# erikszasz/GaussianSplattingRegistration

Measured on AMD Instinct MI355X. Metric: Gaussians/sec through HEM level + ICP iters/sec, 2x5M-splat pair, higher is better.
Workload: dtype f32 (HEM) / f64 (ICP)

## Files before the change

### gaussiansplattingregistration_amd/csrc/hem.hip

```cpp
#include "gsr_common.h"
#include "gsr_math.h"
#include "gsr_normals.h"
#include "gsr_test_hooks.h"
#include "hem_device.h"
#include "hem_select.h"

#include <float.h>
#include <math.h>
#include <stdarg.h>
#include <stdlib.h>
#include <string.h>

#include <chrono>
#include <vector>

#include <rocprim/rocprim.hpp>

namespace gsr {

std::string& last_error() {
    static thread_local std::string s;
    return s;
}
int32_t fail(int32_t code, const char* fmt, ...) {
// ... 183 lines not shown
        const unsigned long long tot = __shfl(incl, 63);
        const unsigned long long cut = tot / 1000ull;
        int cl = 0, ch = 0;
        {
            unsigned long long run = incl - mine;
            for (int b = 0; b < HIST_BINS / 64; ++b) { run += hv[b]; cl += run <= cut ? 1 : 0; }
            run = tot - incl;
            for (int b = HIST_BINS / 64 - 1; b >= 0; --b) { run += hv[b]; ch += run <= cut ? 1 : 0; }
        }
        for (int o = 32; o > 0; o >>= 1) { cl += __shfl_xor(cl, o); ch += __shfl_xor(ch, o); }
        int lo = cl < HIST_BINS - 1 ? cl : HIST_BINS - 1;
        int hi = HIST_BINS - 1 - ch;
        hi = hi > lo ? hi : lo;
        lo = lo > 0 ? lo - 1 : 0;
        hi = hi < HIST_BINS - 1 ? hi + 1 : HIST_BINS - 1;
        const float w = ext / (float)HIST_BINS;
        const float nmn = mn[k] + w * (float)lo, nmx = mn[k] + w * (float)(hi + 1);
        mn[k] = nmn; mx[k] = nmx < mx[k] ? nmx : mx[k];
        inside *= 0.998;
    }
    float ex = mx[0] - mn[0], ey = mx[1] - mn[1], ez = mx[2] - mn[2];
    float emax = fmaxf(ex, fmaxf(ey, ez));
    float eps = emax * 1e-6f + 1e-30f;
    double vol = (double)(ex + eps) * (double)(ey + eps) * (double)(ez + eps);
    double c = cbrt(vol * (double)target / (inside > 1.0 ? inside : 1.0));
    if (!(c > 0.0)) c = 1.0;
    int gx, gy, gz;
    for (;;) {
        double fx = floor(ex / c) + 1.0, fy = floor(ey / c) + 1.0, fz = floor(ez / c) + 1.0;
        if (fx * fy * fz <= (double)max_cells && fx < 2e6 && fy < 2e6 && fz < 2e6) { gx = (int)fx; gy = (int)fy; gz = (int)fz; break; }
        c *= 1.2599210498948732;
    }
    g.ox = mn[0]; g.oy = mn[1]; g.oz = mn[2];
    g.c = (float)c; g.inv_c = 1.0f / g.c;
    g.slack = 1e-5f * (emax + g.c);
    g.gx = gx; g.gy = gy; g.gz = gz; g.ncells = gx * gy * gz;
    if (lane == 0) *gp = g;
}

__global__ __launch_bounds__(256) void k_keys(int64_t n, const float* __restrict__ xyz,
                                              const GridParams* __restrict__ gpp,
                                              unsigned* __restrict__ keys, unsigned* __restrict__ idx) {
    const GridParams g = *gpp;
    for (int64_t i = (int64_t)blockIdx.x * blockDim.x + threadIdx.x; i < n; i += (int64_t)gridDim.x * blockDim.x) {
        int cx = cell_of(xyz[3 * i], g.ox, g.inv_c, g.gx);
        int cy = cell_of(xyz[3 * i + 1], g.oy, g.inv_c, g.gy);
        int cz = cell_of(xyz[3 * i + 2], g.oz, g.inv_c, g.gz);
        keys[i] = (unsigned)((cz * g.gy + cy) * g.gx + cx);
        idx[i] = (unsigned)i;
    }
}

template <typename OffT>
__global__ __launch_bounds__(256) void k_run_starts(int64_t m, const unsigned* __restrict__ skeys, int64_t nkeys,
                                                    OffT* __restrict__ start) {
    for (int64_t j = (int64_t)blockIdx.x * blockDim.x + threadIdx.x; j < m; j += (int64_t)gridDim.x * blockDim.x) {
        unsigned k = skeys[j];
        int64_t prev = j == 0 ? -1 : (int64_t)skeys[j - 1];
        if ((int64_t)k != prev)
            for (int64_t c = prev + 1; c <= (int64_t)k; ++c) start[c] = (OffT)j;
        if (j == m - 1)
            for (int64_t c = (int64_t)k + 1; c <= nkeys; ++c) start[c] = (OffT)m;
    }
}
template <typename OffT>
__global__ void k_fill_const(int64_t n, OffT* p, OffT v) {
    for (int64_t j = (int64_t)blockIdx.x * blockDim.x + threadIdx.x; j < n; j += (int64_t)gridDim.x * blockDim.x) p[j] = v;
}

__global__ __launch_bounds__(256) void k_gather(int64_t n, const unsigned* __restrict__ order, const float4* __restrict__ rec, float delta,
                                                float4* __restrict__ A, float4* __restrict__ geo, float* __restrict__ Rs,
                                                int* __restrict__ pflag, int* __restrict__ iflag,
                                                const float* __restrict__ sh, int F, float* __restrict__ sh_tail ) {
    __shared__ float4 s_t[4][64 * 5];
    float4* st = s_t[threadIdx.x >> 6];
    const int lane = threadIdx.x & 63;
    if (blockIdx.x == 0 && threadIdx.x == 0) iflag[n] = 0;
    if (sh_tail && blockIdx.x == 0)
        for (int t = threadIdx.x; t < ((F + 3) & ~3) + 4; t += blockDim.x) sh_tail[t] = t < F ? sh[(n - 1) * F + t] : 0.0f;
    const int64_t base = (int64_t)blockIdx.x * blockDim.x + (threadIdx.x & ~63);
    if (base < n) {
        const int64_t j = base + lane;
        const unsigned oi = j < n ? order[j] : 0u;
        float4 v[4];
        unsigned iu[4];
#pragma unroll
        for (int u = 0; u < 4; ++u) {
            iu[u] = (unsigned)__shfl((int)oi, (lane >> 2) + 16 * u, 64);
            v[u] = rec[4 * (int64_t)iu[u] + (lane & 3)];
        }
        asm volatile("" : "+v"(v[0].x), "+v"(v[0].y), "+v"(v[0].z), "+v"(v[0].w), "+v"(v[1].x), "+v"(v[1].y), "+v"(v[1].z), "+v"(v[1].w),
                          "+v"(v[2].x), "+v"(v[2].y), "+v"(v[2].z), "+v"(v[2].w), "+v"(v[3].x), "+v"(v[3].y), "+v"(v[3].z), "+v"(v[3].w));
        if ((lane & 3) == 0) {
#pragma unroll
            for (int u = 0; u < 4; ++u) v[u].w = __uint_as_float((__float_as_uint(v[u].w) & 3u) | (iu[u] << 2));
        }
#pragma unroll
        for (int u = 0; u < 4; ++u) {
            const int r = (lane >> 2) + 16 * u;
            if (base + r < n) {
                geo[4 * (base + r) + (lane & 3)] = v[u];
                st[r * 5 + (lane & 3)] = v[u];
            }
        }
        __builtin_amdgcn_wave_barrier();
        if (j < n) {
            const float4 a = st[lane * 5], b = st[lane * 5 + 1], cc = st[lane * 5 + 2];
            const unsigned fl = __float_as_uint(a.w);
            A[j] = a;
            float R = 0.0f;
            if (fl & 1u) {
                const s6 cov = {b.x, b.y, b.z, b.w, cc.x, cc.y};
                R = delta * sqrtf(eig_max6(cov));
            }
            Rs[j] = R;
            pflag[j] = (int)(fl & 1u);
            iflag[j] = (fl & 2u) ? 0 : 1;
        }
        __builtin_amdgcn_wave_barrier();
    }
}
struct __attribute__((packed, aligned(4))) f4u { float x, y, z, w; };
__global__ __launch_bounds__(256) void k_gather_sh(int64_t n, int F, int RSH, const unsigned* __restrict__ order,
                                                   const float* __restrict__ sh, float* __restrict__ shs,
                                                   const int64_t* __restrict__ poff, const unsigned* __restrict__ pcnt, int P, int policy, float thr,
                                                   int* __restrict__ mode_out) {
    {
        int direct = policy == 1 ? 1 : 0;
        if (policy == 2) {
            const double pairs = P > 0 ? (double)poff[P - 1] + (double)pcnt[P - 1] : 0.0;
            direct = pairs < (double)thr * (double)n ? 1 : 0;
        }
        if (blockIdx.x == 0 && threadIdx.x == 0) *mode_out = direct;
        if (direct) return;
    }
    const int Q = RSH >> 2;
    const int64_t total = n * Q;
    const int64_t stride = (int64_t)gridDim.x * blockDim.x;
    auto row_piece = [&](int64_t t, int64_t& j, int& q) -> float4 {
        j = total < ((int64_t)1 << 31) ? (int64_t)((unsigned)t / (unsigned)Q) : t / Q;
        q = (int)(t - j * Q);
        const float* src = sh + (int64_t)order[j] * F + 4 * q;
        const int left = F - 4 * q;
        float4 v;
        if (left >= 4) {
            const f4u u = *reinterpret_cast<const f4u*>(src);
            v = make_float4(u.x, u.y, u.z, u.w);
        } else {
            v.x = left > 0 ? src[0] : 0.0f; v.y = left > 1 ? src[1] : 0.0f; v.z = left > 2 ? src[2] : 0.0f; v.w = 0.0f;
        }
        return v;
    };
    int64_t t = (int64_t)blockIdx.x * blockDim.x + threadIdx.x;
    for (; t + stride < total; t += 2 * stride) {
        int64_t j0, j1;
        int q0, q1;
        const float4 v0 = row_piece(t, j0, q0), v1 = row_piece(t + stride, j1, q1);
        reinterpret_cast<float4*>(shs + j0 * RSH)[q0] = v0;
        reinterpret_cast<float4*>(shs + j1 * RSH)[q1] = v1;
    }
    if (t < total) {
        int64_t j0;
        int q0;
        const float4 v0 = row_piece(t, j0, q0);
        reinterpret_cast<float4*>(shs + j0 * RSH)[q0] = v0;
    }
}
__global__ __launch_bounds__(256) void k_scatter_list(int64_t n, const int* __restrict__ flag, const int* __restrict__ pos,
                                                      unsigned* __restrict__ list) {
    for (int64_t j = (int64_t)blockIdx.x * blockDim.x + threadIdx.x; j < n; j += (int64_t)gridDim.x * blockDim.x)
        if (flag[j]) list[pos[j]] = (unsigned)j;
}

__global__ __launch_bounds__(256) void k_child_stream(int64_t n, int64_t cells, int P, const float4* __restrict__ A, const int* __restrict__ pflag,
                                                      const int* __restrict__ ppos, const int* __restrict__ cellStart,
                                                      float4* __restrict__ Ac, int* __restrict__ cellStartC, int pad,
                                                      const int* __restrict__ irank , int* __restrict__ cellStartI) {
    const int64_t stride = (int64_t)gridDim.x * blockDim.x, t0 = (int64_t)blockIdx.x * blockDim.x + threadIdx.x;
    for (int64_t t = t0; t < pad; t += stride) Ac[(n - P) + t] = make_float4(0.0f, 0.0f, 0.0f, 0.0f);
    for (int64_t j = t0; j < n; j += stride) {
        if (pflag[j]) continue;
        const float4 a = A[j];
        Ac[j - ppos[j]] = make_float4(a.x, a.y, a.z, __uint_as_float(((unsigned)j << 2) | (__float_as_uint(a.w) & 3u)));
    }
    for (int64_t cidx = t0; cidx <= cells; cidx += stride) {
        const int sidx = cellStart[cidx];
        cellStartC[cidx] = sidx - (sidx < n ? ppos[sidx] : P);
        if (irank) cellStartI[cidx] = irank[sidx];
    }
}

#ifndef ORDER_AXIS_BITS
#define ORDER_AXIS_BITS 6
#endif
#ifndef ORDER_FINE_FROM
#define ORDER_FINE_FROM 1000000
#endif
__host__ __device__ inline int order_axis_bits(int P) { return P >= ORDER_FINE_FROM ? ORDER_AXIS_BITS : 3; }
__host__ __device__ inline int order_drop_bits(int P) { return P >= ORDER_FINE_FROM ? 0 : 1; }
__host__ __device__ inline int order_key_bits(int P) { return 3 * order_axis_bits(P) - order_drop_bits(P); }
__global__ __launch_bounds__(1024) void k_heavy_items(int P, const unsigned* __restrict__ sorted_keys, int* __restrict__ nheavy_p,
                                                      const unsigned* __restrict__ porder,
                                                      const unsigned* __restrict__ pcap, const int64_t* __restrict__ coff, unsigned* __restrict__ part_out,
                                                      int own_lo, int own_hi, int first_pull, int max_items,
                                                      uint2* __restrict__ hitem, int* __restrict__ hfirst, unsigned* __restrict__ pcnt,
                                                      int* __restrict__ hq, int* __restrict__ error_flag) {
    __shared__ int s_wsum[16];
    __shared__ int s_base, s_nheavy;
    unsigned part = SEL_PART;
    {
        const unsigned long long cand = (unsigned long long)coff[P - 1] + pcap[P - 1];
        while (part > 2048u && (unsigned long long)part * 4ull * 7168ull > cand) part >>= 1;
    }
    if (threadIdx.x == 0) {
        *part_out = part;
        int lo = 0, hi = P;
        while (lo < hi) { const int mid = (lo + hi) >> 1; if (sorted_keys[mid] >= (3u << order_key_bits(P))) hi = mid; else lo = mid + 1; }
        s_nheavy = lo;
        *nheavy_p = lo;
        s_base = 0;
    }
    __syncthreads();
    const int nheavy = s_nheavy;
    const int lane = threadIdx.x & 63, wv = threadIdx.x >> 6;
    for (int h0 = 0; h0 < nheavy; h0 += 1024) {
        const int h = h0 + (int)threadIdx.x;
        int p = -1, np = 0;
        if (h < nheavy) {
            p = (int)porder[h];
            if (p >= own_lo && p < own_hi) { const unsigned c = pcap[p]; np = (int)(c / part + (c % part ? 1u : 0u)); np = np < 1 ? 1 : np; }
        }
        int incl = np;
        for (int o = 1; o < 64; o <<= 1) { const int v = __shfl_up(incl, o, 64); if (lane >= o) incl += v; }
        if (lane == 63) s_wsum[wv] = incl;
// ... 1457 lines not shown
        const int64_t row0 = t * a.tile;
        const int nrows = (int)(n_pre - row0 < a.tile ? n_pre - row0 : a.tile);
        const int k0 = holes_below(s_holes, d, row0), k1 = holes_below(s_holes, d, row0 + nrows);
        if (k1 == 0) continue;
        const int kn = row0 + nrows < n_pre ? k1 : 0;
        const int tail0 = nrows - kn;
        __syncthreads();
        if ((int)threadIdx.x < nrows) {
            const int64_t r = row0 + threadIdx.x;
            int k = 0; bool hole = false;
            for (int i = 0; i < d; ++i) { k += (int64_t)s_holes[i] < r ? 1 : 0; hole = hole || (int64_t)s_holes[i] == r; }
            s_k[threadIdx.x] = hole ? (short)-1 : (short)(k - k0);
        }
        __syncthreads();
        const int ndst = nrows - (k1 - k0);
        const float* hn = a.halo + (t + 1) * ERASE_MAX * a.W;
        int off = 0;
        for (int q = 0; q < 6; ++q) {
            const int w = a.w[q];
            if (w > 0) {
                float* arr = a.arr[q];
                for (unsigned e = threadIdx.x; e < (unsigned)(nrows * w); e += blockDim.x) {
                    const unsigned rl = e / (unsigned)w, cc = e - rl * (unsigned)w;
                    const int kk = s_k[rl];
                    if (kk < 0) continue;
                    const float v = (int)rl >= tail0 ? hn[off + ((int)rl - tail0) * w + cc] : arr[(row0 + rl) * w + cc];
                    s_stage[((int)rl - kk) * w + cc] = v;
                }
                __syncthreads();
                for (int e = threadIdx.x; e < ndst * w; e += blockDim.x) arr[(row0 - k0) * w + e] = s_stage[e];
                __syncthreads();
            }
            off += ERASE_MAX * w;
        }
        {
            uint8_t* sb = reinterpret_cast<uint8_t*>(s_stage);
            if ((int)threadIdx.x < nrows && s_k[threadIdx.x] >= 0) {
                const int rl = threadIdx.x;
                sb[rl - s_k[rl]] = rl >= tail0 ? halo_b[(t + 1) * ERASE_MAX + (rl - tail0)] : a.flags[row0 + rl];
            }
            __syncthreads();
            if ((int)threadIdx.x < ndst) a.flags[row0 - k0 + threadIdx.x] = sb[threadIdx.x];
            __syncthreads();
        }
    }
}

__global__ void k_level_tail(int64_t n, int P, const int* __restrict__ orank_in, const int* __restrict__ oflag_in, long long out_cap,
                             long long* __restrict__ lvl, int* __restrict__ abort_p) {
    long long n_orph = (long long)orank_in[n - 1] + oflag_in[n - 1];
    if ((long long)P + n_orph > out_cap) { *abort_p = 1; n_orph = out_cap > P ? out_cap - P : 0; }
    lvl[0] = (long long)P + n_orph;
    lvl[1] = n_orph;
}

struct LevelCollect {
    const int64_t* coff; const unsigned* pcap;
    const int64_t* poff; const unsigned* pcnt;
    int P;
    const int* cnt;
    const long long* lvl;
    const GridParams* gp; const unsigned* bbox;
};
enum { LC_CAND = 0, LC_PAIRS, LC_ORPHANS, LC_NPRE, LC_FLAGS, LC_HEAVY, LC_ITEMS, LC_MAXPAIRS, LC_DROPPED, LC_NEXT_P, LC_NEXT_IRR, LC_NEXT_GP, LC_WORDS = 16 };
__global__ void k_level_collect(LevelCollect q, unsigned long long* __restrict__ dst, unsigned long long seq) {
    const int t = threadIdx.x;
    unsigned long long v = 0ull;
    const bool sel = q.P > 0 && q.coff != nullptr;
    if (t == LC_CAND) v = sel ? (unsigned long long)q.coff[q.P - 1] + q.pcap[q.P - 1] : 0ull;
    else if (t == LC_PAIRS) v = sel ? (unsigned long long)q.poff[q.P - 1] + q.pcnt[q.P - 1] : 0ull;
    else if (t == LC_ORPHANS) v = q.lvl ? (unsigned long long)q.lvl[1] : 0ull;
    else if (t == LC_NPRE) v = q.lvl ? (unsigned long long)q.lvl[0] : 0ull;
    else if (t == LC_FLAGS) v = (q.cnt[2] ? 1ull : 0ull) | (q.cnt[12] ? 2ull : 0ull) | (q.cnt[13] ? 4ull : 0ull);
    else if (t == LC_HEAVY) v = (unsigned)q.cnt[8];
    else if (t == LC_ITEMS) v = (unsigned)q.cnt[10];
    else if (t == LC_MAXPAIRS) v = (unsigned)q.cnt[15];
    else if (t == LC_DROPPED) v = (unsigned)q.cnt[3];
    else if (t == LC_NEXT_P) v = q.bbox[6];
    else if (t == LC_NEXT_IRR) v = q.bbox[7];
    else if (t < LC_WORDS) v = reinterpret_cast<const unsigned long long*>(q.gp)[t - LC_NEXT_GP];
    if (t < LC_WORDS) __hip_atomic_store(dst + 16 + t, v, __ATOMIC_RELAXED, __HIP_MEMORY_SCOPE_SYSTEM);
    __threadfence_system();
    __syncthreads();
    if (t == 0) __hip_atomic_store(dst + 15, seq, __ATOMIC_RELEASE, __HIP_MEMORY_SCOPE_SYSTEM);
}
__global__ __launch_bounds__(256) void k_compact_rows(int64_t n, int width, const int* __restrict__ keep,
                                                      const int* __restrict__ pos, const float* __restrict__ src,
                                                      float* __restrict__ dst) {
    const int64_t total = n * width;
    for (int64_t t = (int64_t)blockIdx.x * blockDim.x + threadIdx.x; t < total; t += (int64_t)gridDim.x * blockDim.x) {
        const int64_t i = t / width;
        if (keep[i]) dst[(int64_t)pos[i] * width + (t - i * width)] = src[t];
    }
}
__global__ __launch_bounds__(256) void k_compact_rows4(int64_t n, int width, const int* __restrict__ keep,
                                                       const int* __restrict__ pos, const float* __restrict__ src,
                                                       float* __restrict__ dst) {
    const int Q = (width + 3) >> 2;
    const int64_t total = n * Q;
    for (int64_t t = (int64_t)blockIdx.x * blockDim.x + threadIdx.x; t < total; t += (int64_t)gridDim.x * blockDim.x) {
        const int64_t i = total < ((int64_t)1 << 31) ? (int64_t)((unsigned)t / (unsigned)Q) : t / Q;
        if (!keep[i]) continue;
        const int q = (int)(t - i * Q);
        const float* s4 = src + i * width + 4 * q;
        float* d4 = dst + (int64_t)pos[i] * width + 4 * q;
        const int left = width - 4 * q;
// ... 967 lines not shown
        long long dg = 0;
        GSR_HIP(hipMemcpyAsync(&dg, c->pcounts.p, 8, hipMemcpyDeviceToHost, st));
        GSR_HIP(hipStreamSynchronize(st));
        if (dg > 0) {
            const int64_t words = (n_pre_glob + 31) / 32 + 1;
            GSR_TRY(c->gbits.reserve((size_t)words * 4)); GSR_TRY(c->wcnt.reserve((size_t)words * 4)); GSR_TRY(c->wpre.reserve((size_t)words * 4));
            GSR_HIP(hipMemsetAsync(c->gbits.p, 0, (size_t)words * 4, st));
            if (n_pre > 0) {
                GSR_TRY(c->scratch.reserve((size_t)n_pre * 4));
                hipLaunchKernelGGL(k_not_flag, dim3(stride_grid(n_pre)), blk, 0, st, n_pre, c->keep.as<int>(), c->scratch.as<int>());
                hipLaunchKernelGGL(k_bits_set, dim3(stride_grid(n_pre)), blk, 0, st, n_pre, c->gid_next.as<unsigned>(), c->scratch.as<int>(), c->gbits.as<unsigned>());
            }
            GSR_TRY(gsr_comm_allreduce(c->comm, c->gbits.p, words, GSR_DT_U32, GSR_OP_SUM, (void*)st));
            hipLaunchKernelGGL(k_bits_popc, dim3(stride_grid(words)), blk, 0, st, words, c->gbits.as<unsigned>(), c->wcnt.as<int>());
            GSR_TRY(exclusive_scan<int>(c, c->wcnt.as<int>(), c->wpre.as<int>(), words));
            if (dropped > 0) {
                GSR_TRY(c->grank.reserve((size_t)n_pre * 4));
                hipLaunchKernelGGL(k_compact_u32, dim3(stride_grid(n_pre)), blk, 0, st, n_pre, c->keep.as<int>(), c->kpos.as<int>(), c->gid_next.as<unsigned>(), c->grank.as<unsigned>());
                c->gid_next.swap(c->grank);
            }
            if (O.n > 0) hipLaunchKernelGGL(k_gid_drop, dim3(stride_grid(O.n)), blk, 0, st, O.n, c->gbits.as<unsigned>(), c->wpre.as<int>(), c->gid_next.as<unsigned>());
            n_glob_next = n_pre_glob - dg;
        }
        c->part_stats[6] = dg;
        return GSR_OK;
    }
};

}

namespace {

constexpr int32_t GSR_RETRY_SYNC = -1000;

struct LevelRun {
    gsr_hem_ctx* c;
    hipStream_t st;
    Level& L;
    Level& O;
    const bool dbg_sync, part, sharded;
    bool spec = false;
    const int sh_policy;
    const int64_t n_own;
    int64_t n;
    const int F, RSH;
    PartLevel pl;
    const dim3 blk{256};
    dim3 grd;
    GridParams gp;
    int P_all = 0, P = 0, n_irr = 0;
    int* cnt = nullptr;
    long long* lvl = nullptr;
    const float4* rec_src = nullptr;
    bool ranks_forked = false, sh_pending = false, sh_launched = false, flags_forked = false;
    SelectArgs sa;
    size_t Pm = 1;
    int own_lo = 0, own_hi = 0;
    int64_t M = 0;
    unsigned long long cand = 0, cap_pairs = 0;
    const int64_t* seg = nullptr;
    const unsigned* pc = nullptr;
    const float* pw = nullptr;
    int bshift = 0, nbuckets = 0;
    int* overflow_flag = nullptr;
    bool fixed_tried = false;
    int64_t n_orph = 0, n_pre = 0, out_cap = 0;
    bool out_active = false;
    uint64_t rng_pos0 = 0;
    int64_t dropped = 0, P_glob = 0, O_glob = 0, n_pre_glob = 0, n_glob_next = 0;
    float pro_ms = 0.0f;

    LevelRun(gsr_hem_ctx* ctx, bool allow_async)
        : c(ctx), st(ctx->stream), L(ctx->cur), O(ctx->nxt), dbg_sync(getenv("GSR_HEM_DEBUG_SYNC") != nullptr), part(ctx->comm != nullptr),
          sharded(ctx->shard_world > 1 && ctx->shard_allreduce != nullptr), sh_policy(ctx->comm == nullptr ? ctx->sh_policy : 0), n_own(ctx->cur.n), n(ctx->cur.n), F(ctx->cur.F), RSH((ctx->cur.F + 3) & ~3) {
        spec = allow_async;
        pl.c = c; pl.st = st; pl.n_own = n_own;
        memset(&sa, 0, sizeof(sa));
    }
    ~LevelRun() {
        if (out_active) for (int i = 0; i < 5; ++i) { DevBuf* b = level_big(c->nxt, i); b->p = nullptr; b->cap = 0; b->swap(c->spare_out[i]); }
    }

    int32_t run(int64_t* n_out, int64_t* n_dropped);
    int32_t grid_phase();
    int32_t select_phase();
    int32_t sums_phase();
    int32_t sums_fixed();
    int32_t sums_exact();
    int32_t compact_pairs();
    int32_t output_ranks();
    int32_t open_output();
    int32_t mstep_phase();
    int32_t flags_and_validity();
    int32_t compact_erased(int64_t n_keep);
    int32_t erase_in_place(int64_t rows_bound, bool may_allocate, int64_t alloc_rows = 0);
    bool erase_on_device = false;
    int32_t launch_gather_sh(bool fork);
    int32_t widen_scan(const unsigned* cnt_in, int64_t* off, int64_t count);
    int32_t total_of(const int64_t* off, const unsigned* cnt_in, int64_t count, int64_t* out);
};

struct WidenU32 { __device__ __host__ int64_t operator()(unsigned v) const { return (int64_t)v; } };
int32_t LevelRun::widen_scan(const unsigned* cnt_in, int64_t* off, int64_t count) {
    auto in = rocprim::make_transform_iterator(cnt_in, WidenU32());
    size_t bytes = 0;
    if (count >= GSR_SCAN_BIG_N) {
        GSR_HIP(rocprim::exclusive_scan<scan_cfg64_big>(nullptr, bytes, in, off, (int64_t)0, (size_t)count, rocprim::plus<int64_t>(), st));
// ... 30 lines not shown
                           c->ghost_sh.as<float>(), c->shs.as<float>());
    else
        hipLaunchKernelGGL(k_gather_sh, dim3(shg), blk, 0, sst, n, F, RSH, c->order.as<unsigned>(), L.sh.as<float>(), c->shs.as<float>(),
                           P > 0 ? c->poff.as<int64_t>() : (const int64_t*)nullptr, c->pcnt.as<unsigned>(), P, sh_policy, c->sh_direct_pairs,
                           reinterpret_cast<int*>(lvl + 3));
    if (fork) { GSR_HIP(hipEventRecord(c->ev_sh_join, c->aux2)); sh_pending = true; }
    return GSR_OK;
}

int32_t LevelRun::grid_phase() {
    GSR_TRY(c->counters.reserve(128)); GSR_TRY(c->lvl.reserve(64));
    lvl = c->lvl.as<long long>();
    if (!part && !sharded) {
        if (!(c->pro.valid && c->pro.n == n)) GSR_TRY(prologue_now(c));
        if (!c->pro.valid) return fail(GSR_E_INVALID, "gsr_hem_run_level: no prologue for the level");
        gp = c->pro.gp; P_all = c->pro.P; n_irr = c->pro.n_irr; c->cblock = c->pro.cblock; pro_ms = c->pro.ms;
        c->pro.valid = false;
        cnt = c->counters.as<int>() + 16 * c->cblock;
    } else {
        c->pro.valid = false;
        c->cblock ^= 1;
        cnt = c->counters.as<int>() + 16 * c->cblock;
        GSR_TRY(c->rec.reserve(n * 64)); GSR_TRY(c->bbox.reserve(64));
        GSR_TRY(c->gparams.reserve(sizeof(GridParams)));
        GSR_TRY(c->bbox_part.reserve((size_t)grd.x * 8 * 4)); GSR_TRY(c->hist.reserve(3 * HIST_BINS * 4));
        hipLaunchKernelGGL(k_prep, grd, blk, 0, st, n, L.xyz.as<float>(), L.color.as<float>(), L.cov6.as<float>(), L.opacity.as<float>(),
                           L.weight.as<float>(), L.is_parent.as<uint8_t>(), c->rec.as<float4>(), c->bbox_part.as<unsigned>(), (const long long*)nullptr);
        hipLaunchKernelGGL(k_bbox_reduce, dim3(1), dim3(256), 0, st, (int)grd.x, c->bbox_part.as<unsigned>(), c->bbox.as<unsigned>(),
                           (unsigned*)cnt, 16, c->hist.as<unsigned>(), 3 * HIST_BINS, (unsigned*)nullptr, 0);
        if (part) {
            hipLaunchKernelGGL(k_flip3, dim3(1), dim3(64), 0, st, c->bbox.as<unsigned>());
            GSR_TRY(gsr_comm_allreduce(c->comm, c->bbox.p, 6, GSR_DT_U32, GSR_OP_MAX, (void*)st));
            hipLaunchKernelGGL(k_flip3, dim3(1), dim3(64), 0, st, c->bbox.as<unsigned>());
        }
        hipLaunchKernelGGL(k_hist, dim3(stride_grid(n) > 512 ? 512 : stride_grid(n)), blk, 0, st, n, L.xyz.as<float>(), c->bbox.as<unsigned>(), c->hist.as<unsigned>(),
                           (const long long*)nullptr);
        if (part) GSR_TRY(gsr_comm_allreduce(c->comm, c->hist.p, 3 * HIST_BINS, GSR_DT_U32, GSR_OP_SUM, (void*)st));
        hipLaunchKernelGGL(k_grid_params, dim3(1), dim3(64), 0, st, c->bbox.as<unsigned>(), c->hist.as<unsigned>(), part ? c->n_global : n, c->cell_target,
                           c->max_cells, c->gparams.as<GridParams>(), (const long long*)nullptr);
        static_assert(sizeof(GridParams) == 40, "GridParams is read back as five 8-byte words");
        Collect q;
        q.n = 7;
        for (int i = 0; i < 5; ++i) { q.src[i] = (const char*)c->gparams.p + 8 * i; q.bytes[i] = 8; }
        q.src[5] = c->bbox.as<unsigned>() + 6; q.src[6] = c->bbox.as<unsigned>() + 7;
        q.bytes[5] = q.bytes[6] = 4;
        unsigned long long w[8];
        GSR_TRY(read_back(c, q, w));
        memcpy(&gp, w, sizeof(gp));
        P_all = (int)(unsigned)w[5]; n_irr = (int)(unsigned)w[6];
    }
    overflow_flag = cnt + 12;
    c->stats[5] = gp.ncells;
    GSR_TRY(c->pflag_in.reserve(n * 4)); GSR_TRY(c->oflag_in.reserve(n * 4)); GSR_TRY(c->prank_in.reserve(n * 4)); GSR_TRY(c->orank_in.reserve(n * 4));
    if (!part && c->aux && c->ev_pre) {
        GSR_HIP(hipEventRecord(c->ev_fork, st)); GSR_HIP(hipStreamWaitEvent(c->aux, c->ev_fork, 0));
        hipLaunchKernelGGL(k_flags_in, grd, blk, 0, c->aux, n, n_own, L.is_parent.as<uint8_t>(), c->pflag_in.as<int>(), c->oflag_in.as<int>());
        GSR_TRY(exclusive_scan<int>(c, c->pflag_in.as<int>(), c->prank_in.as<int>(), n, true));
        GSR_HIP(hipEventRecord(c->ev_pre, c->aux));
        ranks_forked = true;
    }

    rec_src = c->rec.as<float4>();
    if (part) {
        GSR_TRY(pl.halo(gp, L, F, n));
        grd = dim3(stride_grid(n));
        rec_src = c->rec_loc.as<float4>();
    }
    GSR_TRY(c->keys.reserve(n * 4)); GSR_TRY(c->idx.reserve(n * 4)); GSR_TRY(c->skeys.reserve(n * 4)); GSR_TRY(c->order.reserve(n * 4));
    if (part) {
        GSR_TRY(c->perm.reserve(n * 4));
        hipLaunchKernelGGL(k_iota, grd, blk, 0, st, n, c->idx.as<unsigned>());
        GSR_TRY(sort_pairs<unsigned>(c, c->gid_loc.as<unsigned>(), c->skeys.as<unsigned>(), c->idx.as<unsigned>(), c->perm.as<unsigned>(), n, bits_for(c->n_global + 1)));
        hipLaunchKernelGGL(k_keys_rec, grd, blk, 0, st, n, rec_src, c->perm.as<unsigned>(), c->gparams.as<GridParams>(), c->keys.as<unsigned>(), c->idx.as<unsigned>());
    } else
        hipLaunchKernelGGL(k_keys, grd, blk, 0, st, n, L.xyz.as<float>(), c->gparams.as<GridParams>(), c->keys.as<unsigned>(), c->idx.as<unsigned>());
    GSR_TRY(sort_pairs<unsigned>(c, c->keys.as<unsigned>(), c->skeys.as<unsigned>(), c->idx.as<unsigned>(), c->order.as<unsigned>(), n,
                                 bits_for(gp.ncells)));
    GSR_TRY(c->cellStart.reserve(((size_t)gp.ncells + 1) * 4));
    hipLaunchKernelGGL(k_run_starts<int>, grd, blk, 0, st, n, c->skeys.as<unsigned>(), (int64_t)gp.ncells, c->cellStart.as<int>());

    GSR_TRY(c->A.reserve((n + SEL_PAD) * 16)); GSR_TRY(c->geo.reserve((size_t)n * 64));
    if (sh_policy != 1) GSR_TRY(c->shs.reserve((size_t)n * (RSH > 0 ? RSH : 1) * 4));
    GSR_TRY(c->Rs.reserve(n * 4)); GSR_TRY(c->pflag.reserve(n * 4));
    GSR_TRY(c->iflag.reserve((n + 1) * 4)); GSR_TRY(c->irank.reserve((n + 1) * 4)); GSR_TRY(c->ipos.reserve(n * 4)); GSR_TRY(c->ppos.reserve(n * 4)); GSR_TRY(c->plist.reserve(n * 4));
    const bool tail = !part && F > 0;
    if (tail) GSR_TRY(c->sh_tail.reserve((size_t)(RSH + 4) * 4));
    hipLaunchKernelGGL(k_gather, dim3((unsigned)((n + 255) / 256)), blk, 0, st, n, c->order.as<unsigned>(), rec_src, c->delta, c->A.as<float4>(), c->geo.as<float4>(),
                       c->Rs.as<float>(), c->pflag.as<int>(), c->iflag.as<int>(), L.sh.as<float>(), F, tail ? c->sh_tail.as<float>() : (float*)nullptr);
    if (part && F > 0) {
        hipLaunchKernelGGL(k_fill_const<int>, dim3(1), dim3(1), 0, st, (int64_t)1, reinterpret_cast<int*>(lvl + 3), 0);
        GSR_TRY(launch_gather_sh(true)); sh_launched = true;
    }
    GSR_TRY(exclusive_scan<int>(c, c->pflag.as<int>(), c->ppos.as<int>(), n));
    if (part) {
        GSR_TRY(c->pown.reserve(n * 4)); GSR_TRY(c->ppos_own.reserve(n * 4)); GSR_TRY(c->inv.reserve(n * 4));
        hipLaunchKernelGGL(k_own_flags, grd, blk, 0, st, n, n_own, c->order.as<unsigned>(), c->pflag.as<int>(), c->pown.as<int>(), c->inv.as<unsigned>());
        GSR_TRY(exclusive_scan<int>(c, c->pown.as<int>(), c->ppos_own.as<int>(), n));
        hipLaunchKernelGGL(k_scatter_list, grd, blk, 0, st, n, c->pown.as<int>(), c->ppos_own.as<int>(), c->plist.as<unsigned>());
    } else
        hipLaunchKernelGGL(k_scatter_list, grd, blk, 0, st, n, c->pflag.as<int>(), c->ppos.as<int>(), c->plist.as<unsigned>());
    if (part || n_irr > 0) {
        GSR_TRY(exclusive_scan<int>(c, c->iflag.as<int>(), c->irank.as<int>(), n + 1));
        hipLaunchKernelGGL(k_scatter_list, grd, blk, 0, st, n, c->iflag.as<int>(), c->irank.as<int>(), c->ipos.as<unsigned>());
    }
    P = P_all;
    if (part) {
        Collect q;
        q.n = 5;
        q.src[0] = c->irank.as<int>() + n; q.src[1] = c->ppos.as<int>() + (n - 1); q.src[2] = c->pflag.as<int>() + (n - 1);
        q.src[3] = c->ppos_own.as<int>() + (n - 1); q.src[4] = c->pown.as<int>() + (n - 1);
        for (int i = 0; i < 5; ++i) q.bytes[i] = 4;
        unsigned long long w[8];
        GSR_TRY(read_back(c, q, w));
        n_irr = (int)w[0];
        P_all = (int)w[1] + (int)w[2];
        P = (int)w[3] + (int)w[4];
    }
    c->stats[0] = P;
    c->stats_ex[0] = n_irr;
    GSR_TRY(c->Ac.reserve(((size_t)(n - P_all) + SEL_PAD) * 16)); GSR_TRY(c->cellStartC.reserve(((size_t)gp.ncells + 1) * 4));
    const bool have_irr = part || n_irr > 0;
    if (have_irr) GSR_TRY(c->cellStartI.reserve(((size_t)gp.ncells + 1) * 4));
    hipLaunchKernelGGL(k_child_stream, grd, blk, 0, st, n, (int64_t)gp.ncells, P_all, c->A.as<float4>(), c->pflag.as<int>(), c->ppos.as<int>(),
                       c->cellStart.as<int>(), c->Ac.as<float4>(), c->cellStartC.as<int>(), (int)SEL_PAD,
                       have_irr ? c->irank.as<int>() : (const int*)nullptr, c->cellStartI.as<int>());
    GSR_CHECKPOINT("grid + gather");
    GSR_TIME(c->ev[1], st);
    return GSR_OK;
}

int32_t LevelRun::select_phase() {
    Pm = (size_t)(P > 0 ? P : 1);
    GSR_TRY(c->pcnt.reserve(Pm * 4)); GSR_TRY(c->pcap.reserve(Pm * 4)); GSR_TRY(c->poff.reserve((Pm + 1) * 8));
    GSR_TRY(c->scratch.reserve((Pm * 2 + 128) * 8));
    sa.A = c->A.as<float4>(); sa.geo = c->geo.as<float4>();
    sa.Rs = c->Rs.as<float>(); sa.plist = c->plist.as<unsigned>(); sa.cellStart = c->cellStart.as<int>();
    sa.gp = c->gparams.as<GridParams>(); sa.P = P;
    sa.Ac = c->Ac.as<float4>(); sa.cellStartC = c->cellStartC.as<int>(); sa.cellStartI = c->cellStartI.as<int>();
    sa.irank = c->irank.as<int>(); sa.ipos = c->ipos.as<unsigned>(); sa.n_irr = n_irr; sa.ell = c->use_ell ? 1 : 0;
    own_lo = sharded ? (int)((int64_t)P * c->shard_rank / c->shard_world) : 0;
    own_hi = sharded ? (int)((int64_t)P * (c->shard_rank + 1) / c->shard_world) : P;
    sa.own_lo = own_lo; sa.own_hi = own_hi;
    {
        const float t = c->kappa * c->kappa * 0.5f;
        float x;
        if (t != t) x = t;
        else if (t < 0.0f) x = -1.0f;
        else if (t > FLT_MAX) x = t;
        else {
            x = t * t;
            if (x > FLT_MAX) x = FLT_MAX;
            while (x < FLT_MAX && sqrtf(nextafterf(x, INFINITY)) <= t) x = nextafterf(x, INFINITY);
            while (x > 0.0f && sqrtf(x) > t) x = nextafterf(x, -INFINITY);
        }
        sa.colorThr2 = x;
    }
    sa.kldThr = c->delta * c->delta * 0.5f;
    sa.tau2 = c->tau * c->tau;
    sa.pcnt = c->pcnt.as<unsigned>();
    sa.pcap = c->pcap.as<unsigned>();
    sa.part_p = reinterpret_cast<const unsigned*>(lvl + 2);
    sa.abort_p = cnt + 2;
    sa.np = c->select_np > 0 ? c->select_np : (P >= SEL_NP * 7168 ? SEL_NP : (P >= 2 * 7168 ? 2 : 1));
    M = 0;
    constexpr int WPB = SEL_WPB;
#define GSR_LAUNCH_SELECT(MODE) GSR_TRY(launch_select(MODE, sa, st, c->aux, c->ev_fork, c->ev_join))
    c->sparse_path = false;
    if (P > 0) {
        GSR_TRY(c->prec.reserve(Pm * sizeof(ParentRec)));
        launch_parent_prep(st, P, c->plist.as<unsigned>(), c->geo.as<float4>(), c->Rs.as<float>(), sa.kldThr, sa.ell, c->prec.as<ParentRec>());
        sa.prec = c->prec.as<ParentRec>();
        if (c->use_rowlist && Pm * 2 * SEL_ROWS * sizeof(int2) <= c->rowlist_max) {
            GSR_TRY(c->rowlist.reserve(Pm * 2 * SEL_ROWS * sizeof(int2)));
            sa.rowlist = c->rowlist.as<int2>();
        }
        launch_spans(st, sa);
        GSR_TRY(c->coff.reserve((Pm + 1) * 8));
        GSR_TRY(widen_scan(c->pcap.as<unsigned>(), c->coff.as<int64_t>(), P));
// ... 326 lines not shown
            hipLaunchKernelGGL(k_mstep_heavy_finish, dim3(256), dim3(64), 0, st, ma);                                    \
        }                                                                                                                \
    }
        GSR_TIME1(c->evm[0], st);
        if (nq == 0) { GSR_LAUNCH_MSTEP(0) }
        else if (nq <= 1 * MSTEP_NV) { GSR_LAUNCH_MSTEP(1) }
        else if (nq <= 2 * MSTEP_NV) { GSR_LAUNCH_MSTEP(2) }
        else if (nq <= 4 * MSTEP_NV) { GSR_LAUNCH_MSTEP(4) }
        else if (nq <= 8 * MSTEP_NV) { GSR_LAUNCH_MSTEP(8) }
        else if (nq <= 16 * MSTEP_NV) { GSR_LAUNCH_MSTEP(16) }
        else { GSR_LAUNCH_MSTEP(32) }
#undef GSR_LAUNCH_MSTEP
        if (msplit && hst != st) GSR_HIP(hipStreamWaitEvent(st, c->ev_mjoin, 0));
        GSR_TIME1(c->evm[1], st);
    }
    hipLaunchKernelGGL(k_orphan_rows, dim3(stride_grid(n_own)), blk, 0, st, n_own, P, c->oflag_in.as<int>(), c->orank_in.as<int>(), L.xyz.as<float>(), L.color.as<float>(),
                       L.cov6.as<float>(), L.opacity.as<float>(), L.weight.as<float>(), L.sh.as<float>(), F, O.xyz.as<float>(), O.color.as<float>(),
                       O.cov6.as<float>(), O.opacity.as<float>(), O.weight.as<float>(), O.sh.as<float>(), (int64_t)(spec ? out_cap : n_pre));
    if (sharded && P > 0) {
        const int W = c->shard_world, RW = 14 + F;
        const int chunk = (P + W - 1) / W + 1;
        const size_t chunk_bytes = (size_t)chunk * RW * 4;
        GSR_TRY(c->shard_send.reserve(chunk_bytes)); GSR_TRY(c->shard_recv.reserve(chunk_bytes * W));
        const int own_cnt = own_hi - own_lo;
        if (own_cnt > 0)
            hipLaunchKernelGGL((k_shard_rows<true>), dim3(stride_grid((int64_t)own_cnt * RW)), blk, 0, st, own_lo, own_cnt, F, c->plist.as<unsigned>(),
                               c->order.as<unsigned>(), c->prank_in.as<int>(), c->shard_send.as<float>(), O.xyz.as<float>(), O.color.as<float>(),
                               O.cov6.as<float>(), O.opacity.as<float>(), O.weight.as<float>(), O.sh.as<float>());
        GSR_HIP(hipStreamSynchronize(st));
        if (c->shard_allgather(c->shard_send.p, c->shard_recv.p, (int64_t)chunk_bytes, c->shard_user) != 0)
            return fail(GSR_E_INVALID, "gsr_hem_run_level: all-gather callback failed (merged components)");
        for (int r = 0; r < W; ++r) {
            if (r == c->shard_rank) continue;
            const int lo = (int)((int64_t)P * r / W), hi = (int)((int64_t)P * (r + 1) / W);
            if (hi > lo)
                hipLaunchKernelGGL((k_shard_rows<false>), dim3(stride_grid((int64_t)(hi - lo) * RW)), blk, 0, st, lo, hi - lo, F, c->plist.as<unsigned>(),
                                   c->order.as<unsigned>(), c->prank_in.as<int>(), c->shard_recv.as<float>() + (size_t)r * chunk * RW, O.xyz.as<float>(),
                                   O.color.as<float>(), O.cov6.as<float>(), O.opacity.as<float>(), O.weight.as<float>(), O.sh.as<float>());
        }
    }
    P_glob = P; O_glob = n_orph;
    if (part) GSR_TRY(pl.global_ranks(P, n_pre, P_glob, O_glob));
    n_pre_glob = P_glob + O_glob;
    GSR_CHECKPOINT("M-step + orphans");
    GSR_TIME(c->ev[4], st);
    return GSR_OK;
}

int32_t LevelRun::erase_in_place(int64_t rows_bound, bool may_allocate, int64_t alloc_rows) {
    const int tile0 = std::min(256, 12288 / std::max(F, 6));
    const auto halo_bytes = [&](int64_t rows) { return (size_t)((rows + tile0 - 1) / tile0 + 1) * ERASE_MAX * ((size_t)(14 + F) * 4 + 1) + 64; };
    {
        const size_t need = halo_bytes(rows_bound);
        if (!may_allocate && c->erase_halo.cap < need) {
            hipLaunchKernelGGL(k_fill_const<long long>, dim3(1), dim3(1), 0, st, (int64_t)1, lvl + 4, (long long)0);
            return GSR_OK;
        }
    }
    erase_on_device = true;
    EraseArgs ea;
    memset(&ea, 0, sizeof(ea));
    float* arrs[6] = {O.xyz.as<float>(), O.color.as<float>(), O.cov6.as<float>(), O.opacity.as<float>(), O.weight.as<float>(), O.sh.as<float>()};
    const int ws[6] = {3, 3, 6, 1, 1, F};
    for (int q = 0; q < 6; ++q) { ea.arr[q] = arrs[q]; ea.w[q] = ws[q]; }
    ea.flags = O.is_parent.as<uint8_t>();
    ea.W = 14 + F;
    ea.tile = std::min(256, 12288 / std::max(F, 6));
    ea.max_tiles = (int)((rows_bound + ea.tile - 1) / ea.tile) + 1;
    GSR_TRY(c->erase_halo.reserve(halo_bytes(std::max(rows_bound, alloc_rows))));
    ea.halo = c->erase_halo.as<float>();
    ea.holes = c->holes.as<int>(); ea.dropped = cnt + 3; ea.n_pre_p = lvl; ea.n_keep_out = lvl + 4;
    const int g = std::min(ea.max_tiles, 2048);
    hipLaunchKernelGGL(k_erase_save, dim3(g), blk, 0, st, ea);
    hipLaunchKernelGGL(k_erase_shift, dim3(g), blk, (size_t)12288 * 4, st, ea);
    GSR_HIP(hipGetLastError());
    return GSR_OK;
}

int32_t LevelRun::compact_erased(int64_t n_keep) {
    Level& T = c->tmp;
    const dim3 g2(stride_grid(n_pre));
    GSR_TRY(T.reserve(n_keep, F));
    T.n = n_keep; T.F = F;
    const int* keep = c->keep.as<int>();
    const int* pos = c->kpos.as<int>();
    hipLaunchKernelGGL(k_compact_rows, dim3(stride_grid(n_pre * 3)), blk, 0, st, n_pre, 3, keep, pos, O.xyz.as<float>(), T.xyz.as<float>());
    hipLaunchKernelGGL(k_compact_rows, dim3(stride_grid(n_pre * 3)), blk, 0, st, n_pre, 3, keep, pos, O.color.as<float>(), T.color.as<float>());
    hipLaunchKernelGGL(k_compact_rows, dim3(stride_grid(n_pre * 6)), blk, 0, st, n_pre, 6, keep, pos, O.cov6.as<float>(), T.cov6.as<float>());
    hipLaunchKernelGGL(k_compact_rows, g2, blk, 0, st, n_pre, 1, keep, pos, O.opacity.as<float>(), T.opacity.as<float>());
    hipLaunchKernelGGL(k_compact_rows, g2, blk, 0, st, n_pre, 1, keep, pos, O.weight.as<float>(), T.weight.as<float>());
    if (F > 0)
        hipLaunchKernelGGL(k_compact_rows4, dim3(stride_grid(n_pre * ((F + 3) / 4))), blk, 0, st, n_pre, F, keep, pos, O.sh.as<float>(), T.sh.as<float>());
    hipLaunchKernelGGL(k_compact_bytes, g2, blk, 0, st, n_pre, keep, pos, O.is_parent.as<uint8_t>(), T.is_parent.as<uint8_t>());
    if (out_active) {
        const size_t row_bytes[5] = {12, 12, 24, 4, (size_t)F * 4};
        for (int i = 0; i < 5; ++i)
            if (row_bytes[i] > 0 && n_keep > 0)
                GSR_HIP(hipMemcpyAsync(level_big(O, i)->p, level_big(T, i)->p, (size_t)n_keep * row_bytes[i], hipMemcpyDeviceToDevice, st));
        O.weight.swap(T.weight); O.is_parent.swap(T.is_parent);
        O.n = n_keep;
    } else
        O.swap(T);
    return GSR_OK;
}

int32_t LevelRun::flags_and_validity() {
    if (part) {
        GSR_TRY(c->allflags.reserve((size_t)(n_pre_glob > 0 ? n_pre_glob : 1)));
        GSR_TRY(draw_flags_raw(c, n_pre_glob, c->allflags.as<uint8_t>()));
        if (n_pre > 0)
// ... 355 lines not shown
```

Measured before the change: 570.2 million.

## Fuse run-starts into gather, scatter plist in child stream, launch keys earlier

Folds the cell run-start computation into the gather kernel and writes the parent list from the child-stream kernel, which removes two separate kernel launches and their passes over memory. The key-computation kernel is now launched right after the fork event, before the aux-stream work is queued, so it can overlap with the flag scan. The lvl[4] zeroing moves from a single-thread fill launch into the level-tail kernel. The cost is more work per thread in gather and child_stream, plus a dependence on ordering, since plist and cellStart must be ready before the kernels that consume them.

```diff
diff --git a/gaussiansplattingregistration_amd/csrc/hem.hip b/gaussiansplattingregistration_amd/csrc/hem.hip
--- a/gaussiansplattingregistration_amd/csrc/hem.hip
+++ b/gaussiansplattingregistration_amd/csrc/hem.hip
@@ -259,16 +259,19 @@
 }
 
 template <typename OffT>
+__device__ __forceinline__ void run_starts_at(int64_t j, int64_t m, const unsigned* __restrict__ skeys, int64_t nkeys, OffT* __restrict__ start) {
+    unsigned k = skeys[j];
+    int64_t prev = j == 0 ? -1 : (int64_t)skeys[j - 1];
+    if ((int64_t)k != prev)
+        for (int64_t c = prev + 1; c <= (int64_t)k; ++c) start[c] = (OffT)j;
+    if (j == m - 1)
+        for (int64_t c = (int64_t)k + 1; c <= nkeys; ++c) start[c] = (OffT)m;
+}
+template <typename OffT>
 __global__ __launch_bounds__(256) void k_run_starts(int64_t m, const unsigned* __restrict__ skeys, int64_t nkeys,
                                                     OffT* __restrict__ start) {
-    for (int64_t j = (int64_t)blockIdx.x * blockDim.x + threadIdx.x; j < m; j += (int64_t)gridDim.x * blockDim.x) {
-        unsigned k = skeys[j];
-        int64_t prev = j == 0 ? -1 : (int64_t)skeys[j - 1];
-        if ((int64_t)k != prev)
-            for (int64_t c = prev + 1; c <= (int64_t)k; ++c) start[c] = (OffT)j;
-        if (j == m - 1)
-            for (int64_t c = (int64_t)k + 1; c <= nkeys; ++c) start[c] = (OffT)m;
-    }
+    for (int64_t j = (int64_t)blockIdx.x * blockDim.x + threadIdx.x; j < m; j += (int64_t)gridDim.x * blockDim.x)
+        run_starts_at<OffT>(j, m, skeys, nkeys, start);
 }
 template <typename OffT>
 __global__ void k_fill_const(int64_t n, OffT* p, OffT v) {
@@ -278,7 +281,8 @@
 __global__ __launch_bounds__(256) void k_gather(int64_t n, const unsigned* __restrict__ order, const float4* __restrict__ rec, float delta,
                                                 float4* __restrict__ A, float4* __restrict__ geo, float* __restrict__ Rs,
                                                 int* __restrict__ pflag, int* __restrict__ iflag,
-                                                const float* __restrict__ sh, int F, float* __restrict__ sh_tail ) {
+                                                const float* __restrict__ sh, int F, float* __restrict__ sh_tail ,
+                                                const unsigned* __restrict__ skeys, int64_t ncells, int* __restrict__ cellStart) {
     __shared__ float4 s_t[4][64 * 5];
     float4* st = s_t[threadIdx.x >> 6];
     const int lane = threadIdx.x & 63;
@@ -289,6 +293,7 @@
     if (base < n) {
         const int64_t j = base + lane;
         const unsigned oi = j < n ? order[j] : 0u;
+        if (j < n) run_starts_at<int>(j, n, skeys, ncells, cellStart);
         float4 v[4];
         unsigned iu[4];
 #pragma unroll
@@ -382,11 +387,15 @@
 __global__ __launch_bounds__(256) void k_child_stream(int64_t n, int64_t cells, int P, const float4* __restrict__ A, const int* __restrict__ pflag,
                                                       const int* __restrict__ ppos, const int* __restrict__ cellStart,
                                                       float4* __restrict__ Ac, int* __restrict__ cellStartC, int pad,
-                                                      const int* __restrict__ irank , int* __restrict__ cellStartI) {
+                                                      const int* __restrict__ irank , int* __restrict__ cellStartI,
+                                                      unsigned* __restrict__ plist ) {
     const int64_t stride = (int64_t)gridDim.x * blockDim.x, t0 = (int64_t)blockIdx.x * blockDim.x + threadIdx.x;
     for (int64_t t = t0; t < pad; t += stride) Ac[(n - P) + t] = make_float4(0.0f, 0.0f, 0.0f, 0.0f);
     for (int64_t j = t0; j < n; j += stride) {
-        if (pflag[j]) continue;
+        if (pflag[j]) {
+            if (plist) plist[ppos[j]] = (unsigned)j;
+            continue;
+        }
         const float4 a = A[j];
         Ac[j - ppos[j]] = make_float4(a.x, a.y, a.z, __uint_as_float(((unsigned)j << 2) | (__float_as_uint(a.w) & 3u)));
     }
@@ -1950,6 +1959,7 @@
     if ((long long)P + n_orph > out_cap) { *abort_p = 1; n_orph = out_cap > P ? out_cap - P : 0; }
     lvl[0] = (long long)P + n_orph;
     lvl[1] = n_orph;
+    lvl[4] = 0;
 }
 
 struct LevelCollect {
@@ -3023,7 +3033,7 @@
     int* cnt = nullptr;
     long long* lvl = nullptr;
     const float4* rec_src = nullptr;
-    bool ranks_forked = false, sh_pending = false, sh_launched = false, flags_forked = false;
+    bool keys_launched = false, ranks_forked = false, sh_pending = false, sh_launched = false, flags_forked = false;
     SelectArgs sa;
     size_t Pm = 1;
     int own_lo = 0, own_hi = 0;
@@ -3160,8 +3170,12 @@
     overflow_flag = cnt + 12;
     c->stats[5] = gp.ncells;
     GSR_TRY(c->pflag_in.reserve(n * 4)); GSR_TRY(c->oflag_in.reserve(n * 4)); GSR_TRY(c->prank_in.reserve(n * 4)); GSR_TRY(c->orank_in.reserve(n * 4));
+    GSR_TRY(c->keys.reserve(n * 4)); GSR_TRY(c->idx.reserve(n * 4));
     if (!part && c->aux && c->ev_pre) {
-        GSR_HIP(hipEventRecord(c->ev_fork, st)); GSR_HIP(hipStreamWaitEvent(c->aux, c->ev_fork, 0));
+        GSR_HIP(hipEventRecord(c->ev_fork, st));
+        hipLaunchKernelGGL(k_keys, grd, blk, 0, st, n, L.xyz.as<float>(), c->gparams.as<GridParams>(), c->keys.as<unsigned>(), c->idx.as<unsigned>());
+        keys_launched = true;
+        GSR_HIP(hipStreamWaitEvent(c->aux, c->ev_fork, 0));
         hipLaunchKernelGGL(k_flags_in, grd, blk, 0, c->aux, n, n_own, L.is_parent.as<uint8_t>(), c->pflag_in.as<int>(), c->oflag_in.as<int>());
         GSR_TRY(exclusive_scan<int>(c, c->pflag_in.as<int>(), c->prank_in.as<int>(), n, true));
         GSR_HIP(hipEventRecord(c->ev_pre, c->aux));
@@ -3180,12 +3194,11 @@
         hipLaunchKernelGGL(k_iota, grd, blk, 0, st, n, c->idx.as<unsigned>());
         GSR_TRY(sort_pairs<unsigned>(c, c->gid_loc.as<unsigned>(), c->skeys.as<unsigned>(), c->idx.as<unsigned>(), c->perm.as<unsigned>(), n, bits_for(c->n_global + 1)));
         hipLaunchKernelGGL(k_keys_rec, grd, blk, 0, st, n, rec_src, c->perm.as<unsigned>(), c->gparams.as<GridParams>(), c->keys.as<unsigned>(), c->idx.as<unsigned>());
-    } else
+    } else if (!keys_launched)
         hipLaunchKernelGGL(k_keys, grd, blk, 0, st, n, L.xyz.as<float>(), c->gparams.as<GridParams>(), c->keys.as<unsigned>(), c->idx.as<unsigned>());
     GSR_TRY(sort_pairs<unsigned>(c, c->keys.as<unsigned>(), c->skeys.as<unsigned>(), c->idx.as<unsigned>(), c->order.as<unsigned>(), n,
                                  bits_for(gp.ncells)));
     GSR_TRY(c->cellStart.reserve(((size_t)gp.ncells + 1) * 4));
-    hipLaunchKernelGGL(k_run_starts<int>, grd, blk, 0, st, n, c->skeys.as<unsigned>(), (int64_t)gp.ncells, c->cellStart.as<int>());
 
     GSR_TRY(c->A.reserve((n + SEL_PAD) * 16)); GSR_TRY(c->geo.reserve((size_t)n * 64));
     if (sh_policy != 1) GSR_TRY(c->shs.reserve((size_t)n * (RSH > 0 ? RSH : 1) * 4));
@@ -3194,7 +3207,8 @@
     const bool tail = !part && F > 0;
     if (tail) GSR_TRY(c->sh_tail.reserve((size_t)(RSH + 4) * 4));
     hipLaunchKernelGGL(k_gather, dim3((unsigned)((n + 255) / 256)), blk, 0, st, n, c->order.as<unsigned>(), rec_src, c->delta, c->A.as<float4>(), c->geo.as<float4>(),
-                       c->Rs.as<float>(), c->pflag.as<int>(), c->iflag.as<int>(), L.sh.as<float>(), F, tail ? c->sh_tail.as<float>() : (float*)nullptr);
+                       c->Rs.as<float>(), c->pflag.as<int>(), c->iflag.as<int>(), L.sh.as<float>(), F, tail ? c->sh_tail.as<float>() : (float*)nullptr,
+                       c->skeys.as<unsigned>(), (int64_t)gp.ncells, c->cellStart.as<int>());
     if (part && F > 0) {
         hipLaunchKernelGGL(k_fill_const<int>, dim3(1), dim3(1), 0, st, (int64_t)1, reinterpret_cast<int*>(lvl + 3), 0);
         GSR_TRY(launch_gather_sh(true)); sh_launched = true;
@@ -3205,8 +3219,7 @@
         hipLaunchKernelGGL(k_own_flags, grd, blk, 0, st, n, n_own, c->order.as<unsigned>(), c->pflag.as<int>(), c->pown.as<int>(), c->inv.as<unsigned>());
         GSR_TRY(exclusive_scan<int>(c, c->pown.as<int>(), c->ppos_own.as<int>(), n));
         hipLaunchKernelGGL(k_scatter_list, grd, blk, 0, st, n, c->pown.as<int>(), c->ppos_own.as<int>(), c->plist.as<unsigned>());
-    } else
-        hipLaunchKernelGGL(k_scatter_list, grd, blk, 0, st, n, c->pflag.as<int>(), c->ppos.as<int>(), c->plist.as<unsigned>());
+    }
     if (part || n_irr > 0) {
         GSR_TRY(exclusive_scan<int>(c, c->iflag.as<int>(), c->irank.as<int>(), n + 1));
         hipLaunchKernelGGL(k_scatter_list, grd, blk, 0, st, n, c->iflag.as<int>(), c->irank.as<int>(), c->ipos.as<unsigned>());
@@ -3231,7 +3244,7 @@
     if (have_irr) GSR_TRY(c->cellStartI.reserve(((size_t)gp.ncells + 1) * 4));
     hipLaunchKernelGGL(k_child_stream, grd, blk, 0, st, n, (int64_t)gp.ncells, P_all, c->A.as<float4>(), c->pflag.as<int>(), c->ppos.as<int>(),
                        c->cellStart.as<int>(), c->Ac.as<float4>(), c->cellStartC.as<int>(), (int)SEL_PAD,
-                       have_irr ? c->irank.as<int>() : (const int*)nullptr, c->cellStartI.as<int>());
+                       have_irr ? c->irank.as<int>() : (const int*)nullptr, c->cellStartI.as<int>(), part ? (unsigned*)nullptr : c->plist.as<unsigned>());
     GSR_CHECKPOINT("grid + gather");
     GSR_TIME(c->ev[1], st);
     return GSR_OK;
@@ -3664,10 +3677,7 @@
     const auto halo_bytes = [&](int64_t rows) { return (size_t)((rows + tile0 - 1) / tile0 + 1) * ERASE_MAX * ((size_t)(14 + F) * 4 + 1) + 64; };
     {
         const size_t need = halo_bytes(rows_bound);
-        if (!may_allocate && c->erase_halo.cap < need) {
-            hipLaunchKernelGGL(k_fill_const<long long>, dim3(1), dim3(1), 0, st, (int64_t)1, lvl + 4, (long long)0);
-            return GSR_OK;
-        }
+        if (!may_allocate && c->erase_halo.cap < need) return GSR_OK;
     }
     erase_on_device = true;
     EraseArgs ea;
```

Result: no change. 570.1 million (-0.0%).
